# grantjr1842/index-tts

Measured on AMD Instinct MI355X. Metric: synthesised audio seconds per second (IndexTTS-2 infer_v2 hot path), whole job, higher is better.
Workload: dtype f32 (greedy decode + its prefill: exact fp32 MFMA; fp32 accumulate and fp32 activations everywhere) + split-bf16 (fp32 operands as hi+lo bf16, 3 bf16 MFMAs per product) GEMMs, DiT attention and convolutions in s2mel, the latent pass and the vocoder; GPT linear weights STORED as bf16 (rounded once at

## Files before the change

index-tts_amd/csrc/decode.h:

```cpp
#pragma once
#include "common.h"

namespace idxtts {

struct DecodeState {
  int pos;
  int mel_pos;
  int step;
  unsigned arrive;
};

struct SlotState {
  int pos;
  int mel_pos;
  int step;
  int max_step;
  int live;
};

struct DecodeAttnArgs {
  const float* qkv_part = nullptr; int parts = 0; int part_rows = 0;
  const float* qkv_bias = nullptr;
  void* kcache = nullptr; void* vcache = nullptr; int kv16 = 0;
  float* out = nullptr;
  float* out_row = nullptr;
  const int* kstart = nullptr;
  const DecodeState* st = nullptr;
  int B = 0, H = 0, Smax = 0, d = 0;
  float scale = 0.125f;
  int pos_hint = 0;
  int nsplit = 1;
  float* part = nullptr;
  unsigned* cnt = nullptr;
  const SlotState* slot = nullptr;
};
int decode_attn_nsplit(int B, int H);
int decode_attn_forward(const DecodeAttnArgs& a, hipStream_t stream);

struct SampleArgs {
  const float* part = nullptr; int parts = 0; int part_rows = 0;
  const float* bias = nullptr;
  float* logits_out = nullptr;
  unsigned char* seen = nullptr;
  int* finished = nullptr;
  long long* codes = nullptr; int codes_ld = 0;
  int* cur_tok = nullptr;
  const DecodeState* st = nullptr;
  int B = 0, V = 0, stop_token = 0;
  float penalty = 1.0f;
  const long long* forced = nullptr; int forced_ld = 0;
  struct Embed {
    float* x_row = nullptr; float* x_stats = nullptr;
    float* x_frag = nullptr;
    const float* mel_emb = nullptr; const float* mel_pos = nullptr; int d = 0;
    DecodeState* st_rw = nullptr;
  } embed;
};
int sample_greedy_forward(const SampleArgs& a, hipStream_t stream);
int sample_slots_forward(const SampleArgs& a, SlotState* slots, const int* slot_ids, int n, hipStream_t stream);

enum SampleMode { SAMPLE_HF = 1, SAMPLE_ACCEL = 2 };
__host__ __device__ static inline float exp1_draw(const float* noise, unsigned long long seed, size_t idx) {
  if (noise) return noise[idx];
  unsigned long long z = seed + 0x9E3779B97F4A7C15ull * (unsigned long long)(idx + 1);
  z = (z ^ (z >> 30)) * 0xBF58476D1CE4E5B9ull;
  z = (z ^ (z >> 27)) * 0x94D049BB133111EBull;
  z = z ^ (z >> 31);
  const float u = ((float)(z >> 40) + 0.5f) * (1.0f / 16777216.0f);
  return -logf(u);
}
struct SampleWarpArgs {
  SampleArgs base;
  int mode = SAMPLE_HF;
  float temperature = 1.0f;
  int top_k = 0;
  float top_p = 1.0f;
  const float* exp_noise = nullptr;
  unsigned long long seed = 0;
};
int sample_warp_forward(const SampleWarpArgs& a, hipStream_t stream);
struct SlotSampling {
  int mode;
  float temperature;
  int top_k;
  float top_p;
  unsigned long long seed;
  const float* exp_noise;
};
int sample_slots_warp_forward(const SampleArgs& a, SlotState* slots, const SlotSampling* samp, const int* slot_ids, int n,
// ... 48 lines not shown
```

index-tts_amd/csrc/decode.hip:

```cpp
#include <algorithm>
#include <cstdlib>

#include "decode.h"
#include "device_util.h"
#include "prof.h"

namespace idxtts {

__device__ __forceinline__ void decode_attn_finish(const DecodeAttnArgs& p, const int b, const int h, const int z, const int NS, const int tid,
                                                   const float o, const float mx, const float l) {
  const int d = p.d;
  auto put = [&](float val) {
    if (p.out_row) p.out_row[(size_t)b * d + h * 64 + tid] = val;
    else p.out[frag_index(b, h * 64 + tid, d >> 4)] = val;
  };
  if (NS == 1) {
    if (tid < 64) put(l > 0.f ? o / l : 0.f);
    return;
  }
  float* mine = p.part + ((size_t)(b * p.H + h) * NS + z) * 66;
  if (tid < 64) __hip_atomic_store(&mine[tid], o, __ATOMIC_RELAXED, __HIP_MEMORY_SCOPE_AGENT);
  if (tid == 64) __hip_atomic_store(&mine[64], mx, __ATOMIC_RELAXED, __HIP_MEMORY_SCOPE_AGENT);
  if (tid == 65) __hip_atomic_store(&mine[65], l, __ATOMIC_RELAXED, __HIP_MEMORY_SCOPE_AGENT);
  if (!wg_arrive_last(&p.cnt[b * p.H + h], (unsigned)NS) || tid >= 64) return;
  const float* all = p.part + (size_t)(b * p.H + h) * NS * 66;
  float mi[16], li[16], oi[16];
#pragma unroll
  for (int i = 0; i < 16; ++i) {
    const bool on = i < NS;
    mi[i] = on ? __hip_atomic_load(&all[i * 66 + 64], __ATOMIC_RELAXED, __HIP_MEMORY_SCOPE_AGENT) : -1e30f;
    li[i] = on ? __hip_atomic_load(&all[i * 66 + 65], __ATOMIC_RELAXED, __HIP_MEMORY_SCOPE_AGENT) : 0.f;
    oi[i] = on ? __hip_atomic_load(&all[i * 66 + tid], __ATOMIC_RELAXED, __HIP_MEMORY_SCOPE_AGENT) : 0.f;
  }
  float M = -1e30f;
#pragma unroll
  for (int i = 0; i < 16; ++i) M = fmaxf(M, mi[i]);
  float O = 0.f, L = 0.f;
#pragma unroll
  for (int i = 0; i < 16; ++i) {
    const float wgt = li[i] > 0.f ? expf(mi[i] - M) : 0.f;
    O += wgt * oi[i];
    L += wgt * li[i];
  }
  put(L > 0.f ? O / L : 0.f);
}

__device__ __forceinline__ void decode_attn_dead(const DecodeAttnArgs& p, const int b, const int h, const int z, const int tid) {
  if (z != 0 || tid >= 64) return;
  if (p.out_row) p.out_row[(size_t)b * p.d + h * 64 + tid] = 0.f;
  else p.out[frag_index(b, h * 64 + tid, p.d >> 4)] = 0.f;
}

struct KvF32 {
  typedef float E;
  typedef f32x4 G;
  typedef f32x4 Acc;
  typedef f32x4 VNew;
  static constexpr int EPG = 4;
  static constexpr int NACC = 4;
  static constexpr int OUT_UNROLL = 32;
  __device__ static __forceinline__ G zero() { return G{0.f, 0.f, 0.f, 0.f}; }
  __device__ static __forceinline__ float put(E* dst, const bool write, const float x) {
    if (write) *dst = x;
    return x;
  }
  __device__ static __forceinline__ float dot_new(const float (&qv)[64], const float* knew) {
    float dot = 0.f;
#pragma unroll
    for (int i = 0; i < 16; ++i) dot += qv[4 * i] * knew[4 * i] + qv[4 * i + 1] * knew[4 * i + 1] + qv[4 * i + 2] * knew[4 * i + 2] + qv[4 * i + 3] * knew[4 * i + 3];
    return dot;
  }
  __device__ static __forceinline__ float dot_key(const float (&qv)[64], const G (&kk)[16]) {
    float dot = 0.f;
#pragma unroll
    for (int i = 0; i < 16; ++i) dot += qv[4 * i] * kk[i][0] + qv[4 * i + 1] * kk[i][1] + qv[4 * i + 2] * kk[i][2] + qv[4 * i + 3] * kk[i][3];
    return dot;
  }
  __device__ static __forceinline__ VNew vnew_of(const float* vnew, const int l) { return *reinterpret_cast<const f32x4*>(&vnew[4 * l]); }
  __device__ static __forceinline__ void fma(Acc& acc, const float pw, const G v) { acc += pw * v; }
  __device__ static __forceinline__ void fma_new(Acc& acc, const float pw, const VNew vn) { acc += pw * vn; }
  __device__ static __forceinline__ void store(float* dst, const Acc (&a)[4]) { *reinterpret_cast<f32x4*>(dst) = (a[0] + a[1]) + (a[2] + a[3]); }
};
struct KvBf16 {
  typedef unsigned short E;
  typedef u32x4 G;
  struct Acc { float e[8]; };
  typedef const float* VNew;
  static constexpr int EPG = 8;
  static constexpr int NACC = 2;
  static constexpr int OUT_UNROLL = 16;
  __device__ static __forceinline__ G zero() { return G{0u, 0u, 0u, 0u}; }
  __device__ static __forceinline__ float put(E* dst, const bool write, const float x) {
    const unsigned bits = bf16_rne_bits(x);
    if (write) *dst = (unsigned short)bits;
    return __uint_as_float(bits << 16);
  }
  __device__ static __forceinline__ float dot_new(const float (&qv)[64], const float* knew) {
    float dot = 0.f;
#pragma unroll
    for (int i = 0; i < 64; ++i) dot += qv[i] * knew[i];
    return dot;
  }
  __device__ static __forceinline__ float dot_key(const float (&qv)[64], const G (&kk)[8]) {
    float dot = 0.f;
#pragma unroll
    for (int i = 0; i < 8; ++i)
#pragma unroll
      for (int j = 0; j < 4; ++j)
        dot += qv[8 * i + 2 * j] * __uint_as_float(kk[i][j] << 16) + qv[8 * i + 2 * j + 1] * __uint_as_float(kk[i][j] & 0xffff0000u);
    return dot;
  }
  __device__ static __forceinline__ VNew vnew_of(const float* vnew, const int l) { return vnew + 8 * l; }
  __device__ static __forceinline__ void fma(Acc& acc, const float pw, const G v) {
#pragma unroll
    for (int j = 0; j < 4; ++j) {
      acc.e[2 * j] += pw * __uint_as_float(v[j] << 16);
      acc.e[2 * j + 1] += pw * __uint_as_float(v[j] & 0xffff0000u);
    }
  }
  __device__ static __forceinline__ void fma_new(Acc& acc, const float pw, const VNew vn) {
#pragma unroll
    for (int e = 0; e < 8; ++e) acc.e[e] += pw * vn[e];
  }
  __device__ static __forceinline__ void store(float* dst, const Acc (&a)[2]) {
#pragma unroll
    for (int e = 0; e < 8; ++e) dst[e] = a[0].e[e] + a[1].e[e];
  }
};

template <int NT, bool SLOTS, class KV>
__device__ __forceinline__ void decode_attn_body(const DecodeAttnArgs& p) {
  typedef typename KV::G G;
  typedef typename KV::E E;
  constexpr int NW = NT / 64, EPG = KV::EPG, KG = 64 / EPG, LPR = 64 / EPG, NG = NT / LPR, NACC = KV::NACC;
  extern __shared__ __attribute__((aligned(16))) float sm[];
  float* qs = sm;
  float* knew = sm + 64;
  float* vnew = sm + 128;
  float* red = sm + 192;
  float* outp = sm + 256;
  float* pr = sm + 256 + NG * 64;

  const int h = blockIdx.x, b = blockIdx.y, tid = threadIdx.x, wave = tid >> 6, lane = tid & 63;
  int pos;
  if constexpr (SLOTS) {
    if (!p.slot[b].live) { decode_attn_dead(p, b, h, blockIdx.z, tid); return; }
    pos = p.slot[b].pos;
  } else {
    pos = p.st->pos;
  }
  const int d = p.d, Smax = p.Smax;
  G* const kc = static_cast<G*>(p.kcache) + (size_t)(b * p.H + h) * KG * Smax;
  G* const vc = static_cast<G*>(p.vcache) + (size_t)(b * p.H + h) * Smax * LPR;

  const int ks0 = p.kstart ? p.kstart[b] : 0;
  const int NS = gridDim.z, z = blockIdx.z;
  const int chunk = NS > 1 ? (((pos - ks0 + NS) / NS + 15) & ~15) : pos - ks0 + 1;
  const int ks = ks0 + z * chunk;
  const int ke = min(pos, ks + chunk - 1);
  const int grp = tid / LPR, lpr = tid % LPR;
  const int s_first = ks + tid;
  G kk0[KG];
#pragma unroll
  for (int i = 0; i < KG; ++i) kk0[i] = (s_first < pos && s_first <= ke) ? kc[(size_t)i * Smax + s_first] : KV::zero();
  constexpr int VP = 128 / NG;
  G vpre[VP];
#pragma unroll
  for (int j = 0; j < VP; ++j) {
    const int sj = ks + grp + NG * j;
    vpre[j] = (sj < pos && sj <= ke) ? vc[(size_t)sj * LPR + lpr] : KV::zero();
  }

  if (tid < 192) {
    const int which = tid >> 6, dd = tid & 63;
    const int col = which * d + h * 64 + dd;
    const float* row = p.qkv_part + (size_t)b * 3 * d + col;
    const size_t sst = (size_t)p.part_rows * 3 * d;
    float acc = p.qkv_bias ? p.qkv_bias[col] : 0.0f;
    for (int s = 0; s < p.parts; ++s) acc += row[(size_t)s * sst];
    if (which == 0) qs[dd] = acc * p.scale;
    else if (which == 1) knew[dd] = KV::put(reinterpret_cast<E*>(kc + (size_t)(dd / EPG) * Smax + pos) + dd % EPG, z == 0, acc);
    else vnew[dd] = KV::put(reinterpret_cast<E*>(vc + (size_t)pos * LPR) + dd, z == 0, acc);
  }
  __syncthreads();

  const float qlane = qs[lane];
  float qv[64];
#pragma unroll
  for (int i = 0; i < 64; ++i) qv[i] = __int_as_float(__builtin_amdgcn_readlane(__float_as_int(qlane), i));

  float mx = -1e30f;
  if (s_first <= ke) {
    const float dot = s_first == pos ? KV::dot_new(qv, knew) : KV::dot_key(qv, kk0);
    pr[s_first] = dot;
    mx = dot;
  }
  for (int s = s_first + NT; s <= ke; s += NT) {
    float dot;
    if (s == pos) dot = KV::dot_new(qv, knew);
    else {
      G kk[KG];
#pragma unroll
      for (int i = 0; i < KG; ++i) kk[i] = kc[(size_t)i * Smax + s];
      dot = KV::dot_key(qv, kk);
    }
    pr[s] = dot;
    mx = fmaxf(mx, dot);
  }
  mx = wave_max(mx);
  if (lane == 0) red[wave] = mx;
  __syncthreads();
  mx = red[0];
#pragma unroll
  for (int w = 1; w < NW; ++w) mx = fmaxf(mx, red[w]);
  float sum = 0.f;
  for (int s = s_first; s <= ke; s += NT) {
    const float e = expf(pr[s] - mx);
    pr[s] = e;
    sum += e;
  }
  sum = wave_sum(sum);
  if (lane == 0) red[NW + wave] = sum;
  __syncthreads();
  float l = 0.f;
#pragma unroll
  for (int w = 0; w < NW; ++w) l += red[NW + w];

  const typename KV::VNew vn = KV::vnew_of(vnew, lpr);
  typename KV::Acc acc[NACC] = {};
#pragma unroll
  for (int j = 0; j < VP; ++j) {
    const int sj = ks + grp + NG * j;
    if (sj <= ke) {
      if (sj == pos) KV::fma_new(acc[j % NACC], pr[sj], vn);
      else KV::fma(acc[j % NACC], pr[sj], vpre[j]);
    }
  }
  for (int sb = ks + grp + VP * NG; sb <= ke; sb += 8 * NG) {
    G v[8];
#pragma unroll
    for (int j = 0; j < 8; ++j) {
      const int sj = sb + NG * j;
      v[j] = (sj < pos && sj <= ke) ? vc[(size_t)sj * LPR + lpr] : KV::zero();
    }
#pragma unroll
    for (int j = 0; j < 8; ++j) {
      const int sj = sb + NG * j;
      if (sj <= ke) {
        if (sj == pos) KV::fma_new(acc[j % NACC], pr[sj], vn);
        else KV::fma(acc[j % NACC], pr[sj], v[j]);
      }
    }
  }
  KV::store(&outp[grp * 64 + EPG * lpr], acc);
  __syncthreads();
  float o = 0.f;
  if (tid < 64) {
#pragma unroll KV::OUT_UNROLL
    for (int g = 0; g < NG; ++g) o += outp[g * 64 + tid];
  }
  decode_attn_finish(p, b, h, z, NS, tid, o, mx, l);
}

template <int NT, bool SLOTS>
__global__ __launch_bounds__(NT, (NT == 512 ? 4 : 1)) void decode_attn_kernel(const DecodeAttnArgs p) {
  decode_attn_body<NT, SLOTS, KvF32>(p);
}
template <int NT, bool SLOTS>
__global__ __launch_bounds__(NT, (NT == 512 ? 4 : 1)) void decode_attn16_kernel(const DecodeAttnArgs p) {
  decode_attn_body<NT, SLOTS, KvBf16>(p);
}

int decode_attn_nsplit(int B, int H) {
  const int wgs = B * H;
  return wgs <= 128 ? std::max(1, std::min(16, 256 / wgs)) : 1;
}

int decode_attn_forward(const DecodeAttnArgs& a, hipStream_t stream) {
  IDX_CHECK(a.qkv_part && a.kcache && a.vcache && (a.out || a.out_row) && (a.st || a.slot), "null pointer");
  IDX_CHECK(a.d == a.H * 64, "head_dim must be 64");
  constexpr int nt = 512;
  const size_t lds = (size_t)(256 + (nt / (a.kv16 ? 8 : 16)) * 64 + a.Smax) * sizeof(float);
  IDX_CHECK(lds <= 128 * 1024, "Smax too large for the LDS score buffer");
  static DynLdsLimit lds_limit;
  IDX_HIP(lds_limit.set(128 * 1024, decode_attn_kernel<512, false>, decode_attn16_kernel<512, false>, decode_attn_kernel<512, true>, decode_attn16_kernel<512, true>));
  IDX_CHECK(a.nsplit >= 1 && a.nsplit <= 16 && (a.nsplit == 1 || (a.part && a.cnt)), "key split: 1..16 pieces, partial buffer and counters");
  static const int cat = prof_register("decode_attn_kernel"), cat16 = prof_register("decode_attn16_kernel");
  ProfScope prof(a.kv16 ? cat16 : cat, stream, 0.0, (a.kv16 ? 4.0 : 8.0) * a.B * (double)a.pos_hint * a.d);
  const dim3 grid(a.H, a.B, a.nsplit);
  if (a.slot) {
    if (a.kv16) hipLaunchKernelGGL((decode_attn16_kernel<512, true>), grid, dim3(512), lds, stream, a);
    else hipLaunchKernelGGL((decode_attn_kernel<512, true>), grid, dim3(512), lds, stream, a);
  } else {
    if (a.kv16) hipLaunchKernelGGL((decode_attn16_kernel<512, false>), grid, dim3(512), lds, stream, a);
    else hipLaunchKernelGGL((decode_attn_kernel<512, false>), grid, dim3(512), lds, stream, a);
  }
  IDX_LAUNCH_CHECK();
  return 0;
}

__device__ __forceinline__ void greedy_row_argmax(const SampleArgs& p, const int b, const int tid, float* rv, int* ri, float& best_out,
                                                  int& bidx_out) {
  const int wave = tid >> 6, lane = tid & 63;
  const int V = p.V;
  float best = -INFINITY;
  int bidx = 0x7fffffff;
  const unsigned char* seen = p.seen + (size_t)b * V;
  const size_t sst = (size_t)p.part_rows * V;
  const float* prow = p.part + (size_t)b * V;
  for (int v0 = tid; v0 < V; v0 += 4096) {
    float l4[4];
#pragma unroll
    for (int u = 0; u < 4; ++u) {
      const int v = v0 + 1024 * u;
      l4[u] = (v < V && p.bias) ? p.bias[v] : 0.0f;
    }
    for (int s = 0; s < p.parts; ++s) {
#pragma unroll
      for (int u = 0; u < 4; ++u) {
        const int v = v0 + 1024 * u;
        if (v < V) l4[u] += prow[(size_t)s * sst + v];
      }
    }
#pragma unroll
    for (int u = 0; u < 4; ++u) {
      const int v = v0 + 1024 * u;
      if (v >= V) continue;
      float l = l4[u];
      if (p.logits_out) p.logits_out[(size_t)b * V + v] = l;
      if (seen[v]) l = l < 0.f ? l * p.penalty : l / p.penalty;
      if (l > best) { best = l; bidx = v; }
    }
  }
  wave_argmax(best, bidx);
  if (lane == 0) { rv[wave] = best; ri[wave] = bidx; }
  __syncthreads();
  if (tid == 0) argmax_take_waves<16>(best, bidx, rv, ri);
  best_out = best;
  bidx_out = bidx;
}

__device__ __forceinline__ void write_next_input(const SampleArgs& p, const int b, const int tok, const int mel_pos, const int tid) {
  if (p.embed.x_frag) {
    const int d = p.embed.d;
    for (int e = tid; e < d; e += 1024) p.embed.x_frag[frag_index(b, e, d >> 4)] = p.embed.mel_emb[(size_t)tok * d + e] + p.embed.mel_pos[(size_t)mel_pos * d + e];
  } else {
    embed_row_pl<1024>(p.embed.x_row, p.embed.x_stats, b, p.B, p.embed.d, p.embed.mel_emb, p.embed.mel_pos, tok, mel_pos, tid);
  }
// ... 482 lines not shown
```

index-tts_amd/csrc/gpt.hip:

```cpp
#include <algorithm>
#include <cstdlib>
#include <cstring>

#include "gpt.h"
#include "model_util.h"

namespace idxtts {

GPTModel::GPTModel(const idxtts_gpt_config& c) : cfg(c) {}

bool GPTModel::accepts(const std::string& name) const {
  static const char* prefixes[] = {"gpt.h.", "gpt.ln_f.", "final_norm.", "mel_head.", "mel_embedding.", "text_embedding.",
                                   "mel_pos_embedding.", "text_pos_embedding.", "speed_emb."};
  for (const char* p : prefixes)
    if (name.rfind(p, 0) == 0) return true;
  return false;
}

static int upload_stream(DeviceArena& arena, const std::vector<float>& buf, int N, int K, int fmt, Gemv16Weights* gw) {
  gw->N = N; gw->K = K; gw->fmt = fmt;
  if (fmt == WFMT_F32) {
    float* d = nullptr;
    if (arena.upload(buf.data(), buf.size(), &d)) return 1;
    gw->wp = d;
// ... 135 lines not shown
  if (tensor_from(t, arena, "final_norm.weight", {d}, &fn_g) || tensor_from(t, arena, "final_norm.bias", {d}, &fn_b)) return 1;
  const int V = cfg.number_mel_codes;
  HostTensor* hw = nullptr;
  if (need(t, "mel_head.weight", {V, d}, &hw)) return 1;
  std::vector<float> buf(gemv16_packed_floats(V, d));
  pack_gemv16_nk(buf.data(), hw->data.data(), V, d);
  if (upload_stream(arena, buf, V, d, weight_fmt, &head_g)) return 1;
  if (weight_fmt != WFMT_F32 && d % 32 == 0 && upload_stream32(arena, hw->data.data(), V, d, false, weight_fmt, &head_p)) return 1;
  if (tensor_from(t, arena, "mel_head.bias", {V}, &head_b)) return 1;
  if (tensor_from(t, arena, "mel_embedding.weight", {V, d}, &mel_emb)) return 1;
  if (tensor_from(t, arena, "text_embedding.weight", {cfg.number_text_tokens + 1, d}, &text_emb)) return 1;
  if (tensor_from(t, arena, "mel_pos_embedding.emb.weight", {cfg.mel_pos_len, d}, &mel_pos)) return 1;
  if (tensor_from(t, arena, "text_pos_embedding.emb.weight", {cfg.text_pos_len, d}, &text_pos)) return 1;
  return 0;
}

GPTModel::Buffers GPTModel::carve(void* ws, int B, int S, int max_new, size_t prefill_rows) const {
  const int d = cfg.model_dim, V = cfg.number_mel_codes, L = cfg.layers;
  Buffers b;
  Carver c(ws);
  const size_t rows = prefill_rows ? prefill_rows : (size_t)B * S;
  b.x = c.take<float>(rows * d);
  b.h = c.take<float>(rows * d);
  b.qkv = c.take<float>(rows * 3 * d);
  b.att = c.take<float>(rows * d);
  b.ff = c.take<float>(rows * 4 * d);
  b.Smax = max_new > 0 ? ((S + max_new + 3) & ~3) : 0;
  const size_t cache = (size_t)L * kv_layer_bytes(B, b.Smax);
  b.kcache = c.take<char>(cache);
  b.vcache = c.take<char>(cache);
  b.xd = c.take<float>(frag_image_floats(B, d));
  b.frag_off = c.off - frag_image_floats(B, d) * sizeof(float);
  b.hd = c.take<float>(frag_image_floats(B, d));
  b.attd = c.take<float>(frag_image_floats(B, d));
  b.ffd = c.take<float>(frag_image_floats(B, 4 * d));
  b.pl_cnt = c.take<unsigned>((size_t)cdiv(std::max(V, 4 * d), 16));
  b.frag_bytes = c.off - b.frag_off;
  b.xrow = c.take<float>((size_t)B * d);
  b.hrow = c.take<float>((size_t)B * d);
  b.attrow = c.take<float>((size_t)B * d);
  b.ffrow = c.take<float>((size_t)B * 4 * d);
  b.stats = c.take<float>((size_t)cdiv(d, 16) * cdiv(B, 16) * 16 * 2);
  b.pl_slab = c.take<float>(std::max({gemv_pl_slab_floats(3 * d, d, B), gemv_pl_slab_floats(d, d, B), gemv_pl_slab_floats(4 * d, d, B),
                                      gemv_pl_slab_floats(d, 4 * d, B), gemv_pl_slab_floats(V, d, B), (size_t)64}));
  b.qkvd = c.take<float>((size_t)B * 3 * d);
  b.slab = c.take<float>((size_t)8 * B * d);
  b.logits = c.take<float>((size_t)B * V);
  b.seen = c.take<unsigned char>((size_t)B * V);
  b.finished = c.take<int>(B);
  b.cur_tok = c.take<int>(B);
  b.kstart = c.take<int>(B);
  b.ksb_cnt = c.take<unsigned>((size_t)cdiv(d, 16));
  b.attn_cnt = c.take<unsigned>((size_t)B * cfg.heads);
  b.attn_part = c.take<float>((size_t)B * cfg.heads * 16 * 66);
  b.state = c.take<DecodeState>(1);
  b.codes = c.take<long long>((size_t)B * (max_new > 0 ? max_new : 0));
  b.bytes = (c.off + 255) & ~(size_t)255;
  return b;
}

size_t GPTModel::workspace_bytes(int B, int S, int max_new) const { return carve(nullptr, B, S, max_new).bytes; }

int GPTModel::layer_full(int li, const Buffers& w, int B, int S, const int* kstart, bool store_kv, hipStream_t st, const KvScatter* scatter) {
  const bool exact = store_kv && kv_fmt == 0;
  auto mm = [&](const LinearWeights& lw, const GemmArgs& ga) { return exact ? gemm_tn_forward(lw, ga, st) : gemm_forward(lw, ga, st); };
  const GPTLayer& L = layers[li];
  const int d = cfg.model_dim, M = B * S;
  RowsNormArgs n1;
  n1.x_in = w.x; n1.ld_in = d; n1.y = w.h; n1.ld_y = d; n1.M = M; n1.d = d; n1.mode = NORM_LN; n1.g1 = L.ln1_g; n1.b1 = L.ln1_b;
  if (rows_norm_forward(n1, st)) return 1;
  GemmArgs g;
  g.x = w.h; g.ldx = d; g.y = w.qkv; g.ldy = 3 * d; g.M = M;
  if (mm(L.attn_l, g)) return 1;
  if (store_kv && scatter) {
    const size_t per_layer = kv_layer_bytes(scatter->slots, w.Smax);
    if (kv_store_slots(w.qkv, w.kcache + li * per_layer, w.vcache + li * per_layer, kv_fmt, scatter->n, cfg.heads, S, w.Smax, d,
                       scatter->slot_ids, scatter->len, st, scatter->fan)) return 1;
  } else if (store_kv) {
    const size_t per_layer = kv_layer_bytes(B, w.Smax);
    if (kv_store_prefill(w.qkv, w.kcache + li * per_layer, w.vcache + li * per_layer, kv_fmt, B, cfg.heads, S, w.Smax, d, st)) return 1;
  }
  AttnArgs a;
  a.q = w.qkv; a.k = w.qkv + d; a.v = w.qkv + 2 * d; a.o = w.att;
  a.q_bs = a.k_bs = a.v_bs = (long)S * 3 * d; a.o_bs = (long)S * d;
  a.q_ts = a.k_ts = a.v_ts = 3 * d; a.o_ts = d;
  a.B = B; a.H = cfg.heads; a.Sq = S; a.Sk = S; a.causal = 1; a.kstart = kstart; a.scale = 0.125f;
  a.split_bf16 = !exact && get_gemm_mode() == GEMM_BF16X3;
  if (flash_attn_forward(a, st)) return 1;
  GemmArgs p;
  p.x = w.att; p.ldx = d; p.y = w.x; p.ldy = d; p.res = w.x; p.ldr = d; p.M = M;
  if (mm(L.proj_l, p)) return 1;
  RowsNormArgs n2 = n1;
  n2.g1 = L.ln2_g; n2.b1 = L.ln2_b;
  if (rows_norm_forward(n2, st)) return 1;
  GemmArgs f1;
  f1.x = w.h; f1.ldx = d; f1.y = w.ff; f1.ldy = 4 * d; f1.M = M; f1.act = ACT_GELU_NEW;
  if (mm(L.fc_l, f1)) return 1;
  GemmArgs f2;
  f2.x = w.ff; f2.ldx = 4 * d; f2.y = w.x; f2.ldy = d; f2.res = w.x; f2.ldr = d; f2.M = M;
  if (mm(L.fc2_l, f2)) return 1;
  return 0;
}

int GPTModel::head_logits(const Buffers& w, int B, const float* x, int ldx, bool x_frag, hipStream_t st) {
  const int V = cfg.number_mel_codes, d = cfg.model_dim;
  const bool pl = use_pl(B);
  RowsNormArgs n;
// ... 16 lines not shown
int GPTModel::head_and_sample(const Buffers& w, int B, const float* x, int ldx, bool x_frag, float penalty, int codes_ld,
                              float* logits_out, hipStream_t st) {
  const int V = cfg.number_mel_codes, d = cfg.model_dim;
  const bool pl = use_pl(B);
  if (head_logits(w, B, x, ldx, x_frag, st)) return 1;
  if (w.beam_tail) {
    BeamState bs = w.beam;
    bs.penalty = penalty;
    return beam_scores_forward(bs, st) || beam_select_forward(bs, st) || beam_reorder_forward(bs, st);
  }
  SampleArgs s;
  s.part = w.logits; s.parts = 1; s.part_rows = B; s.bias = nullptr; s.logits_out = logits_out;
  s.seen = w.seen; s.finished = w.finished; s.codes = w.codes; s.codes_ld = codes_ld; s.cur_tok = w.cur_tok;
  s.st = w.state; s.B = B; s.V = V; s.stop_token = cfg.stop_mel_token; s.penalty = penalty;
  s.forced = w.forced; s.forced_ld = w.forced_ld;
  if (w.slots) {
    if (pl) { s.embed.x_row = w.xrow; s.embed.x_stats = w.stats; } else s.embed.x_frag = w.xd;
    s.embed.mel_emb = mel_emb; s.embed.mel_pos = mel_pos; s.embed.d = d;
    if (w.slot_samp) return sample_slots_warp_forward(s, w.slots, w.slot_samp, nullptr, B, st);
    return sample_slots_forward(s, w.slots, nullptr, B, st);
  }
  if (fused_tail(w)) {
    if (pl) { s.embed.x_row = w.xrow; s.embed.x_stats = w.stats; } else s.embed.x_frag = w.xd;
    s.embed.mel_emb = mel_emb; s.embed.mel_pos = mel_pos; s.embed.d = d; s.embed.st_rw = w.state;
  }
  if (w.samp.mode != 0) {
    const idxtts_sampling& r = w.samp;
    SampleWarpArgs sw;
    sw.base = s; sw.mode = r.mode; sw.temperature = r.temperature; sw.top_k = r.top_k; sw.top_p = r.top_p;
    sw.exp_noise = r.exp_noise; sw.seed = r.seed;
    return sample_warp_forward(sw, st);
  }
  return sample_greedy_forward(s, st);
}

bool GPTModel::use_pl(int B) const { return weight_fmt != WFMT_F32 && B >= get_decode_plane_rows() && cfg.model_dim % 32 == 0 && head_p.wp; }
bool GPTModel::fused_tail(const Buffers& w) const { return w.slots || (w.samp.mode == 0 && !w.beam_tail); }

int GPTModel::decode_step_pl(const Buffers& w, int B, float penalty, int codes_ld, float* logits_base, int pos_hint, hipStream_t st) {
  const int d = cfg.model_dim, T = d / 16;
  const size_t per_layer = kv_layer_bytes(B, w.Smax);
  const bool fused = fused_tail(w);
  if (!fused && embed_step_pl(w.xrow, w.stats, B, d, mel_emb, mel_pos, w.cur_tok, w.state, st)) return 1;
  for (int li = 0; li < cfg.layers; ++li) {
    const GPTLayer& L = layers[li];
    GemvPLArgs qa;
    qa.x = w.xrow; qa.ldx = d; qa.rows = B; qa.colsum = L.attn_u; qa.bias = L.attn_c; qa.stats_in = w.stats; qa.stats_tiles = T;
    qa.y = w.qkvd; qa.ldy = 3 * d; qa.slab = w.pl_slab; qa.counters = w.pl_cnt;
    if (gemv_pl_forward(L.attn_p, qa, st)) return 1;
    DecodeAttnArgs da;
    da.qkv_part = w.qkvd; da.parts = 1; da.part_rows = B; da.qkv_bias = nullptr;
    da.kcache = w.kcache + li * per_layer; da.vcache = w.vcache + li * per_layer; da.kv16 = kv_fmt; da.out_row = w.attrow; da.kstart = w.kstart;
    da.st = w.state; da.B = B; da.H = cfg.heads; da.Smax = w.Smax; da.d = d; da.scale = 0.125f;
    da.nsplit = decode_attn_nsplit(B, cfg.heads); da.part = w.attn_part; da.cnt = w.attn_cnt; da.slot = w.slots;
    da.pos_hint = pos_hint;
    if (decode_attn_forward(da, st)) return 1;
    GemvPLArgs pa;
    pa.x = w.attrow; pa.ldx = d; pa.rows = B; pa.bias = L.proj_l.bias; pa.res = w.xrow; pa.y = w.xrow; pa.ldy = d; pa.stats_out = w.stats;
    pa.slab = w.pl_slab; pa.counters = w.pl_cnt;
    if (gemv_pl_forward(L.proj_p, pa, st)) return 1;
    GemvPLArgs fa;
    fa.x = w.xrow; fa.ldx = d; fa.rows = B; fa.colsum = L.fc_u; fa.bias = L.fc_c; fa.stats_in = w.stats; fa.stats_tiles = T; fa.act = 1; fa.y = w.ffrow; fa.ldy = 4 * d;
    fa.slab = w.pl_slab; fa.counters = w.pl_cnt;
    if (gemv_pl_forward(L.fc_p, fa, st)) return 1;
    GemvPLArgs fb;
    fb.x = w.ffrow; fb.ldx = 4 * d; fb.rows = B; fb.bias = L.fc2_l.bias; fb.res = w.xrow; fb.y = w.xrow; fb.ldy = d; fb.stats_out = w.stats;
    fb.slab = w.pl_slab; fb.counters = w.pl_cnt;
    if (gemv_pl_forward(L.fc2_p, fb, st)) return 1;
  }
  if (head_and_sample(w, B, w.xrow, d, false, penalty, codes_ld, logits_base, st)) return 1;
  return fused ? 0 : advance_state(w.state, st);
}

int GPTModel::decode_step(const Buffers& w, int B, float penalty, int codes_ld, float* logits_base, int pos_hint, hipStream_t st) {
  if (use_pl(B)) return decode_step_pl(w, B, penalty, codes_ld, logits_base, pos_hint, st);
  const int d = cfg.model_dim;
  const size_t per_layer = kv_layer_bytes(B, w.Smax);
  const bool fused = fused_tail(w);
  if (!fused && embed_step(w.xd, B, d, mel_emb, mel_pos, w.cur_tok, w.state, st)) return 1;
  for (int li = 0; li < cfg.layers; ++li) {
    const GPTLayer& L = layers[li];
    GemvFXArgs qa;
    qa.xf = w.xd; qa.rows = B; qa.colsum = L.attn_u; qa.bias = L.attn_c; qa.y = w.qkvd; qa.ldy = 3 * d;
    if (gemv_fx_forward(L.attn_g, qa, st)) return 1;
    DecodeAttnArgs da;
    da.qkv_part = w.qkvd; da.parts = 1; da.part_rows = B; da.qkv_bias = nullptr;
    da.kcache = w.kcache + li * per_layer; da.vcache = w.vcache + li * per_layer; da.kv16 = kv_fmt; da.out = w.attd; da.kstart = w.kstart;
    da.st = w.state; da.B = B; da.H = cfg.heads; da.Smax = w.Smax; da.d = d; da.scale = 0.125f;
    da.nsplit = decode_attn_nsplit(B, cfg.heads); da.part = w.attn_part; da.cnt = w.attn_cnt; da.slot = w.slots;
    da.pos_hint = pos_hint;
    if (decode_attn_forward(da, st)) return 1;
    GemvFXArgs pa;
    pa.xf = w.attd; pa.rows = B; pa.bias = L.proj_l.bias; pa.res = w.xd; pa.y = w.xd; pa.y_frag = 1;
    if (gemv_fx_forward(L.proj_g, pa, st)) return 1;
    GemvFXArgs fa;
    fa.xf = w.xd; fa.rows = B; fa.colsum = L.fc_u; fa.bias = L.fc_c; fa.act = 1; fa.y = w.ffd; fa.y_frag = 1;
    if (gemv_fx_forward(L.fc_g, fa, st)) return 1;
    GemvFXArgs fb;
    fb.xf = w.ffd; fb.rows = B;
    const int ksb = gemv_fx_ksb(L.fc2_g.N, L.fc2_g.K);
    if (ksb > 1) {
      fb.ksb = ksb; fb.slab = w.slab; fb.ksb_counters = w.ksb_cnt;
      fb.bias = L.fc2_l.bias; fb.res = w.xd; fb.y = w.xd; fb.y_frag = 1;
      if (gemv_fx_forward(L.fc2_g, fb, st)) return 1;
    } else {
      fb.bias = L.fc2_l.bias; fb.res = w.xd; fb.y = w.xd; fb.y_frag = 1;
      if (gemv_fx_forward(L.fc2_g, fb, st)) return 1;
    }
  }
  if (head_and_sample(w, B, w.xd, d, true, penalty, codes_ld, logits_base, st)) return 1;
  return fused ? 0 : advance_state(w.state, st);
}

int GPTModel::capture_step(const Buffers& w, int B, float penalty, int codes_ld, hipStream_t st, StepGraph* g) {
  IDX_HIP(hipStreamBeginCapture(st, hipStreamCaptureModeThreadLocal));
  const int rc = decode_step(w, B, penalty, codes_ld, nullptr, 0, st);
  const hipError_t e = hipStreamEndCapture(st, &g->graph);
  if (rc) return 1;
  IDX_HIP(e);
  IDX_HIP(hipGraphInstantiate(&g->exec, g->graph, nullptr, nullptr, 0));
  return 0;
}

int GPTModel::call_stream(hipStream_t user, hipStream_t* st) {
  *st = user;
  if (user) return 0;
  if (!own_stream) IDX_HIP(hipStreamCreateWithFlags(&own_stream, hipStreamNonBlocking));
  IDX_HIP(hipStreamSynchronize(user));
  *st = own_stream;
  return 0;
}

int GPTModel::run_generation(const Buffers& w, const float* inputs_embeds, const int* pad_left_host, int B, int fan, int P, int max_new,
                             float penalty, float* logits_out, bool graph, hipGraphExec_t exec, StepGraph* captured, const int* poll,
                             int poll_n, int poll_every, int* steps_done, hipStream_t st) {
  const int d = cfg.model_dim, V = cfg.number_mel_codes, S = P + 1, R = B * fan;
  std::vector<int> kstart(R, 0);
  for (int r = 0; r < R; ++r) {
    kstart[r] = pad_left_host ? pad_left_host[r / fan] : 0;
    IDX_CHECK(kstart[r] >= 0 && kstart[r] < P, "pad_left out of range");
  }
  IDX_HIP(hipMemcpyAsync(w.kstart, kstart.data(), R * sizeof(int), hipMemcpyHostToDevice, st));
// ... 433 lines not shown
```

Measured before the change: 188.8.

## Rewrite decode attention as persistent per-wave 64-key chunks with balanced work split

Replaces the per-(head,row,split) workgroup decode attention with a persistent grid sized to the CU count. Each wave handles one 64-key chunk of one (row, head) pair, and the work is balanced across blocks using a prefix sum of live chunk counts per row. Partials are merged by the last-arriving wave through an online softmax. This removes the LDS score buffer and the fixed split heuristic, so the split adapts to each row's actual length and dead slots cost nothing. In exchange it adds per-chunk atomic counters and partial traffic, recomputes q for every chunk, and requires a partial buffer that grows with Smax.

Result: slower. 182.3 (-3.4%).

```diff
diff --git a/index-tts_amd/csrc/decode.h b/index-tts_amd/csrc/decode.h
--- a/index-tts_amd/csrc/decode.h
+++ b/index-tts_amd/csrc/decode.h
@@ -29,12 +29,11 @@
   int B = 0, H = 0, Smax = 0, d = 0;
   float scale = 0.125f;
   int pos_hint = 0;
-  int nsplit = 1;
   float* part = nullptr;
   unsigned* cnt = nullptr;
   const SlotState* slot = nullptr;
 };
-int decode_attn_nsplit(int B, int H);
+size_t decode_attn_part_floats(int B, int H, int Smax);
 int decode_attn_forward(const DecodeAttnArgs& a, hipStream_t stream);
 
 struct SampleArgs {
diff --git a/index-tts_amd/csrc/decode.hip b/index-tts_amd/csrc/decode.hip
--- a/index-tts_amd/csrc/decode.hip
+++ b/index-tts_amd/csrc/decode.hip
@@ -7,99 +7,57 @@
 
 namespace idxtts {
 
-__device__ __forceinline__ void decode_attn_finish(const DecodeAttnArgs& p, const int b, const int h, const int z, const int NS, const int tid,
-                                                   const float o, const float mx, const float l) {
-  const int d = p.d;
-  auto put = [&](float val) {
-    if (p.out_row) p.out_row[(size_t)b * d + h * 64 + tid] = val;
-    else p.out[frag_index(b, h * 64 + tid, d >> 4)] = val;
-  };
-  if (NS == 1) {
-    if (tid < 64) put(l > 0.f ? o / l : 0.f);
-    return;
-  }
-  float* mine = p.part + ((size_t)(b * p.H + h) * NS + z) * 66;
-  if (tid < 64) __hip_atomic_store(&mine[tid], o, __ATOMIC_RELAXED, __HIP_MEMORY_SCOPE_AGENT);
-  if (tid == 64) __hip_atomic_store(&mine[64], mx, __ATOMIC_RELAXED, __HIP_MEMORY_SCOPE_AGENT);
-  if (tid == 65) __hip_atomic_store(&mine[65], l, __ATOMIC_RELAXED, __HIP_MEMORY_SCOPE_AGENT);
-  if (!wg_arrive_last(&p.cnt[b * p.H + h], (unsigned)NS) || tid >= 64) return;
-  const float* all = p.part + (size_t)(b * p.H + h) * NS * 66;
-  float mi[16], li[16], oi[16];
-#pragma unroll
-  for (int i = 0; i < 16; ++i) {
-    const bool on = i < NS;
-    mi[i] = on ? __hip_atomic_load(&all[i * 66 + 64], __ATOMIC_RELAXED, __HIP_MEMORY_SCOPE_AGENT) : -1e30f;
-    li[i] = on ? __hip_atomic_load(&all[i * 66 + 65], __ATOMIC_RELAXED, __HIP_MEMORY_SCOPE_AGENT) : 0.f;
-    oi[i] = on ? __hip_atomic_load(&all[i * 66 + tid], __ATOMIC_RELAXED, __HIP_MEMORY_SCOPE_AGENT) : 0.f;
-  }
-  float M = -1e30f;
-#pragma unroll
-  for (int i = 0; i < 16; ++i) M = fmaxf(M, mi[i]);
-  float O = 0.f, L = 0.f;
-#pragma unroll
-  for (int i = 0; i < 16; ++i) {
-    const float wgt = li[i] > 0.f ? expf(mi[i] - M) : 0.f;
-    O += wgt * oi[i];
-    L += wgt * li[i];
-  }
-  put(L > 0.f ? O / L : 0.f);
-}
-
-__device__ __forceinline__ void decode_attn_dead(const DecodeAttnArgs& p, const int b, const int h, const int z, const int tid) {
-  if (z != 0 || tid >= 64) return;
-  if (p.out_row) p.out_row[(size_t)b * p.d + h * 64 + tid] = 0.f;
-  else p.out[frag_index(b, h * 64 + tid, p.d >> 4)] = 0.f;
-}
+constexpr int DA_NT = 512, DA_NW = DA_NT / 64;
+constexpr int DA_GRAN = 64;
+constexpr int DA_PF = 66;
+constexpr int DA_MAX_ROWS = 512;
+
+size_t decode_attn_part_floats(int B, int H, int Smax) { return (size_t)B * H * cdiv(Smax, DA_GRAN) * DA_PF; }
 
 struct KvF32 {
   typedef float E;
   typedef f32x4 G;
   typedef f32x4 Acc;
-  typedef f32x4 VNew;
   static constexpr int EPG = 4;
-  static constexpr int NACC = 4;
-  static constexpr int OUT_UNROLL = 32;
+  static constexpr int NACC = 2;
+  static constexpr int VPRE = 4;
   __device__ static __forceinline__ G zero() { return G{0.f, 0.f, 0.f, 0.f}; }
-  __device__ static __forceinline__ float put(E* dst, const bool write, const float x) {
-    if (write) *dst = x;
+  __device__ static __forceinline__ float put(E* dst, const float x) {
+    *dst = x;
     return x;
   }
-  __device__ static __forceinline__ float dot_new(const float (&qv)[64], const float* knew) {
-    float dot = 0.f;
-#pragma unroll
-    for (int i = 0; i < 16; ++i) dot += qv[4 * i] * knew[4 * i] + qv[4 * i + 1] * knew[4 * i + 1] + qv[4 * i + 2] * knew[4 * i + 2] + qv[4 * i + 3] * knew[4 * i + 3];
-    return dot;
-  }
+  __device__ static __forceinline__ G pack(const float (&x)[4]) { return G{x[0], x[1], x[2], x[3]}; }
   __device__ static __forceinline__ float dot_key(const float (&qv)[64], const G (&kk)[16]) {
     float dot = 0.f;
 #pragma unroll
     for (int i = 0; i < 16; ++i) dot += qv[4 * i] * kk[i][0] + qv[4 * i + 1] * kk[i][1] + qv[4 * i + 2] * kk[i][2] + qv[4 * i + 3] * kk[i][3];
     return dot;
   }
-  __device__ static __forceinline__ VNew vnew_of(const float* vnew, const int l) { return *reinterpret_cast<const f32x4*>(&vnew[4 * l]); }
   __device__ static __forceinline__ void fma(Acc& acc, const float pw, const G v) { acc += pw * v; }
-  __device__ static __forceinline__ void fma_new(Acc& acc, const float pw, const VNew vn) { acc += pw * vn; }
-  __device__ static __forceinline__ void store(float* dst, const Acc (&a)[4]) { *reinterpret_cast<f32x4*>(dst) = (a[0] + a[1]) + (a[2] + a[3]); }
+  __device__ static __forceinline__ void sum(float (&o)[4], const Acc (&a)[2]) {
+    const f32x4 t = a[0] + a[1];
+#pragma unroll
+    for (int e = 0; e < 4; ++e) o[e] = t[e];
+  }
 };
 struct KvBf16 {
   typedef unsigned short E;
   typedef u32x4 G;
   struct Acc { float e[8]; };
-  typedef const float* VNew;
   static constexpr int EPG = 8;
   static constexpr int NACC = 2;
-  static constexpr int OUT_UNROLL = 16;
+  static constexpr int VPRE = 4;
   __device__ static __forceinline__ G zero() { return G{0u, 0u, 0u, 0u}; }
-  __device__ static __forceinline__ float put(E* dst, const bool write, const float x) {
+  __device__ static __forceinline__ float put(E* dst, const float x) {
     const unsigned bits = bf16_rne_bits(x);
-    if (write) *dst = (unsigned short)bits;
+    *dst = (unsigned short)bits;
     return __uint_as_float(bits << 16);
   }
-  __device__ static __forceinline__ float dot_new(const float (&qv)[64], const float* knew) {
-    float dot = 0.f;
-#pragma unroll
-    for (int i = 0; i < 64; ++i) dot += qv[i] * knew[i];
-    return dot;
+  __device__ static __forceinline__ G pack(const float (&x)[8]) {
+    G g;
+#pragma unroll
+    for (int j = 0; j < 4; ++j) g[j] = (__float_as_uint(x[2 * j]) >> 16) | (__float_as_uint(x[2 * j + 1]) & 0xffff0000u);
+    return g;
   }
   __device__ static __forceinline__ float dot_key(const float (&qv)[64], const G (&kk)[8]) {
     float dot = 0.f;
@@ -110,7 +68,6 @@
         dot += qv[8 * i + 2 * j] * __uint_as_float(kk[i][j] << 16) + qv[8 * i + 2 * j + 1] * __uint_as_float(kk[i][j] & 0xffff0000u);
     return dot;
   }
-  __device__ static __forceinline__ VNew vnew_of(const float* vnew, const int l) { return vnew + 8 * l; }
   __device__ static __forceinline__ void fma(Acc& acc, const float pw, const G v) {
 #pragma unroll
     for (int j = 0; j < 4; ++j) {
@@ -118,182 +75,229 @@
       acc.e[2 * j + 1] += pw * __uint_as_float(v[j] & 0xffff0000u);
     }
   }
-  __device__ static __forceinline__ void fma_new(Acc& acc, const float pw, const VNew vn) {
-#pragma unroll
-    for (int e = 0; e < 8; ++e) acc.e[e] += pw * vn[e];
-  }
-  __device__ static __forceinline__ void store(float* dst, const Acc (&a)[2]) {
-#pragma unroll
-    for (int e = 0; e < 8; ++e) dst[e] = a[0].e[e] + a[1].e[e];
+  __device__ static __forceinline__ void sum(float (&o)[8], const Acc (&a)[2]) {
+#pragma unroll
+    for (int e = 0; e < 8; ++e) o[e] = a[0].e[e] + a[1].e[e];
   }
 };
 
-template <int NT, bool SLOTS, class KV>
+__device__ __forceinline__ void decode_attn_put(const DecodeAttnArgs& p, const int b, const int col, const float val) {
+  if (p.out_row) p.out_row[(size_t)b * p.d + col] = val;
+  else p.out[frag_index(b, col, p.d >> 4)] = val;
+}
+
+template <bool SLOTS, class KV>
 __device__ __forceinline__ void decode_attn_body(const DecodeAttnArgs& p) {
   typedef typename KV::G G;
   typedef typename KV::E E;
-  constexpr int NW = NT / 64, EPG = KV::EPG, KG = 64 / EPG, LPR = 64 / EPG, NG = NT / LPR, NACC = KV::NACC;
-  extern __shared__ __attribute__((aligned(16))) float sm[];
-  float* qs = sm;
-  float* knew = sm + 64;
-  float* vnew = sm + 128;
-  float* red = sm + 192;
-  float* outp = sm + 256;
-  float* pr = sm + 256 + NG * 64;
-
-  const int h = blockIdx.x, b = blockIdx.y, tid = threadIdx.x, wave = tid >> 6, lane = tid & 63;
-  int pos;
-  if constexpr (SLOTS) {
-    if (!p.slot[b].live) { decode_attn_dead(p, b, h, blockIdx.z, tid); return; }
-    pos = p.slot[b].pos;
-  } else {
-    pos = p.st->pos;
-  }
-  const int d = p.d, Smax = p.Smax;
-  G* const kc = static_cast<G*>(p.kcache) + (size_t)(b * p.H + h) * KG * Smax;
-  G* const vc = static_cast<G*>(p.vcache) + (size_t)(b * p.H + h) * Smax * LPR;
-
-  const int ks0 = p.kstart ? p.kstart[b] : 0;
-  const int NS = gridDim.z, z = blockIdx.z;
-  const int chunk = NS > 1 ? (((pos - ks0 + NS) / NS + 15) & ~15) : pos - ks0 + 1;
-  const int ks = ks0 + z * chunk;
-  const int ke = min(pos, ks + chunk - 1);
-  const int grp = tid / LPR, lpr = tid % LPR;
-  const int s_first = ks + tid;
-  G kk0[KG];
-#pragma unroll
-  for (int i = 0; i < KG; ++i) kk0[i] = (s_first < pos && s_first <= ke) ? kc[(size_t)i * Smax + s_first] : KV::zero();
-  constexpr int VP = 128 / NG;
-  G vpre[VP];
-#pragma unroll
-  for (int j = 0; j < VP; ++j) {
-    const int sj = ks + grp + NG * j;
-    vpre[j] = (sj < pos && sj <= ke) ? vc[(size_t)sj * LPR + lpr] : KV::zero();
-  }
-
-  if (tid < 192) {
-    const int which = tid >> 6, dd = tid & 63;
-    const int col = which * d + h * 64 + dd;
-    const float* row = p.qkv_part + (size_t)b * 3 * d + col;
+  constexpr int EPG = KV::EPG, KG = 64 / EPG, LPR = 64 / EPG, NGW = 64 / LPR, NV = DA_GRAN / NGW, NACC = KV::NACC, VPRE = KV::VPRE;
+  static_assert(NGW == EPG, "a lane group's index selects the head dim a lane hands on");
+  __shared__ int s_incl[DA_MAX_ROWS];
+  __shared__ int s_pos[DA_MAX_ROWS];
+  __shared__ int s_ks[DA_MAX_ROWS];
+  const int tid = threadIdx.x, wave = tid >> 6, lane = tid & 63;
+  const int B = p.B, H = p.H, d = p.d, Smax = p.Smax;
+  const int Gmax = (Smax + DA_GRAN - 1) / DA_GRAN;
+
+  if (wave == 0) {
+    int carry = 0;
+    for (int r0 = 0; r0 < B; r0 += 64) {
+      const int r = r0 + lane;
+      int pos = 0, ks0 = 0, g = 0;
+      if (r < B) {
+        bool live = true;
+        ks0 = p.kstart ? p.kstart[r] : 0;
+        if constexpr (SLOTS) { live = p.slot[r].live != 0; pos = p.slot[r].pos; }
+        else pos = p.st->pos;
+        if (live && ks0 >= 0 && pos >= ks0 && pos < Smax) g = (pos - ks0) / DA_GRAN + 1;
+      }
+      int inc = g;
+#pragma unroll
+      for (int off = 1; off < 64; off <<= 1) {
+        const int t = __shfl_up(inc, off);
+        if (lane >= off) inc += t;
+      }
+      inc += carry;
+      if (r < B) { s_incl[r] = inc; s_pos[r] = pos; s_ks[r] = ks0; }
+      carry = __shfl(inc, 63);
+    }
+  }
+  __syncthreads();
+
+  const int T = H * s_incl[B - 1];
+  const int W = min(T, (int)gridDim.x);
+  int run0 = 0, run1 = 0;
+  if ((int)blockIdx.x < W) {
+    run0 = (int)((long long)blockIdx.x * T / W);
+    run1 = (int)((long long)(blockIdx.x + 1) * T / W);
+  }
+
+  for (int f = run0 + wave; f < run1; f += DA_NW) {
+    int b = 0;
+    for (int r0 = 0; r0 < B; r0 += 64) {
+      const int r = r0 + lane;
+      b += __popcll(__ballot(r < B && s_incl[r] * H <= f));
+    }
+    b = __builtin_amdgcn_readfirstlane(b);
+    if (b >= B) break;
+    const int gbase = b ? __builtin_amdgcn_readfirstlane(s_incl[b - 1]) : 0, gb = __builtin_amdgcn_readfirstlane(s_incl[b]) - gbase;
+    if (gb <= 0) break;
+    const int rem = f - gbase * H, h = rem / gb, j = rem - h * gb;
+    const int pos = __builtin_amdgcn_readfirstlane(s_pos[b]);
+    const int gs = __builtin_amdgcn_readfirstlane(s_ks[b]) + DA_GRAN * j;
+    const bool last = j == gb - 1;
+    const int pair = b * H + h;
+    G* const kc = static_cast<G*>(p.kcache) + (size_t)pair * KG * Smax;
+    G* const vc = static_cast<G*>(p.vcache) + (size_t)pair * Smax * LPR;
+    const G* const kg = kc + gs;
+    const G* const vg0 = vc + (size_t)gs * LPR;
+    const int grp = lane / LPR, lpr = lane % LPR;
+    const int s = gs + lane;
+
+    G kk[KG];
+#pragma unroll
+    for (int i = 0; i < KG; ++i) kk[i] = s < pos ? (kg + (size_t)i * Smax)[(unsigned)lane] : KV::zero();
+    G v[NV];
+#pragma unroll
+    for (int jj = 0; jj < VPRE; ++jj) {
+      const int sj = gs + grp + NGW * jj;
+      v[jj] = sj < pos ? (vg0 + NGW * LPR * jj)[(unsigned)lane] : KV::zero();
+    }
+
     const size_t sst = (size_t)p.part_rows * 3 * d;
-    float acc = p.qkv_bias ? p.qkv_bias[col] : 0.0f;
-    for (int s = 0; s < p.parts; ++s) acc += row[(size_t)s * sst];
-    if (which == 0) qs[dd] = acc * p.scale;
-    else if (which == 1) knew[dd] = KV::put(reinterpret_cast<E*>(kc + (size_t)(dd / EPG) * Smax + pos) + dd % EPG, z == 0, acc);
-    else vnew[dd] = KV::put(reinterpret_cast<E*>(vc + (size_t)pos * LPR) + dd, z == 0, acc);
-  }
-  __syncthreads();
-
-  const float qlane = qs[lane];
-  float qv[64];
-#pragma unroll
-  for (int i = 0; i < 64; ++i) qv[i] = __int_as_float(__builtin_amdgcn_readlane(__float_as_int(qlane), i));
-
-  float mx = -1e30f;
-  if (s_first <= ke) {
-    const float dot = s_first == pos ? KV::dot_new(qv, knew) : KV::dot_key(qv, kk0);
-    pr[s_first] = dot;
-    mx = dot;
-  }
-  for (int s = s_first + NT; s <= ke; s += NT) {
-    float dot;
-    if (s == pos) dot = KV::dot_new(qv, knew);
-    else {
-      G kk[KG];
-#pragma unroll
-      for (int i = 0; i < KG; ++i) kk[i] = kc[(size_t)i * Smax + s];
-      dot = KV::dot_key(qv, kk);
-    }
-    pr[s] = dot;
-    mx = fmaxf(mx, dot);
-  }
-  mx = wave_max(mx);
-  if (lane == 0) red[wave] = mx;
-  __syncthreads();
-  mx = red[0];
-#pragma unroll
-  for (int w = 1; w < NW; ++w) mx = fmaxf(mx, red[w]);
-  float sum = 0.f;
-  for (int s = s_first; s <= ke; s += NT) {
-    const float e = expf(pr[s] - mx);
-    pr[s] = e;
-    sum += e;
-  }
-  sum = wave_sum(sum);
-  if (lane == 0) red[NW + wave] = sum;
-  __syncthreads();
-  float l = 0.f;
-#pragma unroll
-  for (int w = 0; w < NW; ++w) l += red[NW + w];
-
-  const typename KV::VNew vn = KV::vnew_of(vnew, lpr);
-  typename KV::Acc acc[NACC] = {};
-#pragma unroll
-  for (int j = 0; j < VP; ++j) {
-    const int sj = ks + grp + NG * j;
-    if (sj <= ke) {
-      if (sj == pos) KV::fma_new(acc[j % NACC], pr[sj], vn);
-      else KV::fma(acc[j % NACC], pr[sj], vpre[j]);
-    }
-  }
-  for (int sb = ks + grp + VP * NG; sb <= ke; sb += 8 * NG) {
-    G v[8];
-#pragma unroll
-    for (int j = 0; j < 8; ++j) {
-      const int sj = sb + NG * j;
-      v[j] = (sj < pos && sj <= ke) ? vc[(size_t)sj * LPR + lpr] : KV::zero();
-    }
-#pragma unroll
-    for (int j = 0; j < 8; ++j) {
-      const int sj = sb + NG * j;
-      if (sj <= ke) {
-        if (sj == pos) KV::fma_new(acc[j % NACC], pr[sj], vn);
-        else KV::fma(acc[j % NACC], pr[sj], v[j]);
-      }
-    }
-  }
-  KV::store(&outp[grp * 64 + EPG * lpr], acc);
-  __syncthreads();
-  float o = 0.f;
-  if (tid < 64) {
-#pragma unroll KV::OUT_UNROLL
-    for (int g = 0; g < NG; ++g) o += outp[g * 64 + tid];
-  }
-  decode_attn_finish(p, b, h, z, NS, tid, o, mx, l);
-}
-
-template <int NT, bool SLOTS>
-__global__ __launch_bounds__(NT, (NT == 512 ? 4 : 1)) void decode_attn_kernel(const DecodeAttnArgs p) {
-  decode_attn_body<NT, SLOTS, KvF32>(p);
-}
-template <int NT, bool SLOTS>
-__global__ __launch_bounds__(NT, (NT == 512 ? 4 : 1)) void decode_attn16_kernel(const DecodeAttnArgs p) {
-  decode_attn_body<NT, SLOTS, KvBf16>(p);
-}
-
-int decode_attn_nsplit(int B, int H) {
-  const int wgs = B * H;
-  return wgs <= 128 ? std::max(1, std::min(16, 256 / wgs)) : 1;
+    const float* row = p.qkv_part + (size_t)b * 3 * d + h * 64 + lane;
+    float qa = p.qkv_bias ? p.qkv_bias[h * 64 + lane] : 0.0f;
+    for (int t = 0; t < p.parts; ++t) qa += row[(size_t)t * sst];
+    const float qlane = qa * p.scale;
+    float klane = 0.f, vlane = 0.f;
+    if (last) {
+      float ka = p.qkv_bias ? p.qkv_bias[d + h * 64 + lane] : 0.0f, va = p.qkv_bias ? p.qkv_bias[2 * d + h * 64 + lane] : 0.0f;
+      for (int t = 0; t < p.parts; ++t) { ka += row[(size_t)t * sst + d]; va += row[(size_t)t * sst + 2 * d]; }
+      klane = KV::put(reinterpret_cast<E*>(kc + (size_t)(lane / EPG) * Smax + pos) + lane % EPG, ka);
+      vlane = KV::put(reinterpret_cast<E*>(vc + (size_t)pos * LPR) + lane, va);
+    }
+    float qv[64];
+#pragma unroll
+    for (int i = 0; i < 64; ++i) qv[i] = __int_as_float(__builtin_amdgcn_readlane(__float_as_int(qlane), i));
+
+    float dot = KV::dot_key(qv, kk);
+    if (last) {
+      const float dn = wave_sum(qlane * klane);
+      if (s == pos) dot = dn;
+    }
+    __builtin_amdgcn_sched_barrier(0);
+#pragma unroll
+    for (int jj = VPRE; jj < NV; ++jj) {
+      const int sj = gs + grp + NGW * jj;
+      v[jj] = sj < pos ? (vg0 + NGW * LPR * jj)[(unsigned)lane] : KV::zero();
+    }
+    const bool on = s <= pos;
+    const float m = wave_max(on ? dot : -1e30f);
+    const float e = on ? expf(dot - m) : 0.f;
+    const float l = wave_sum(e);
+
+    if (last) {
+      float vn[EPG];
+#pragma unroll
+      for (int i = 0; i < EPG; ++i) vn[i] = __shfl(vlane, EPG * lpr + i);
+      const G vg = KV::pack(vn);
+#pragma unroll
+      for (int jj = 0; jj < NV; ++jj)
+        if (gs + grp + NGW * jj == pos) v[jj] = vg;
+    }
+    typename KV::Acc acc[NACC] = {};
+#pragma unroll
+    for (int jj = 0; jj < NV; ++jj) KV::fma(acc[jj % NACC], __shfl(e, grp + NGW * jj), v[jj]);
+    float o[EPG];
+    KV::sum(o, acc);
+#pragma unroll
+    for (int off = LPR; off < 64; off <<= 1)
+#pragma unroll
+      for (int i = 0; i < EPG; ++i) o[i] += __shfl_xor(o[i], off);
+    float mine = o[0];
+#pragma unroll
+    for (int i = 1; i < EPG; ++i) mine = grp == i ? o[i] : mine;
+    const int dd = EPG * lpr + grp;
+
+    if (gb == 1) {
+      decode_attn_put(p, b, h * 64 + dd, l > 0.f ? mine / l : 0.f);
+      continue;
+    }
+    float* const all = p.part + (size_t)pair * Gmax * DA_PF;
+    float* const part = all + (size_t)j * DA_PF;
+    __hip_atomic_store(&part[dd], mine, __ATOMIC_RELAXED, __HIP_MEMORY_SCOPE_AGENT);
+    if (lane == 0) {
+      __hip_atomic_store(&part[64], m, __ATOMIC_RELAXED, __HIP_MEMORY_SCOPE_AGENT);
+      __hip_atomic_store(&part[65], l, __ATOMIC_RELAXED, __HIP_MEMORY_SCOPE_AGENT);
+    }
+    asm volatile("s_waitcnt vmcnt(0)" ::: "memory");
+    int is_last = 0;
+    if (lane == 0) {
+      const unsigned old = __hip_atomic_fetch_add(&p.cnt[pair], 1u, __ATOMIC_RELAXED, __HIP_MEMORY_SCOPE_AGENT);
+      is_last = old == (unsigned)gb - 1u;
+      if (is_last) __hip_atomic_store(&p.cnt[pair], 0u, __ATOMIC_RELAXED, __HIP_MEMORY_SCOPE_AGENT);
+    }
+    is_last = __builtin_amdgcn_readfirstlane(is_last);
+    asm volatile("" ::: "memory");
+    if (!is_last) continue;
+    float M = -1e30f, L = 0.f, O = 0.f;
+    for (int i0 = 0; i0 < gb; i0 += 8) {
+      float mi[8], li[8], oi[8];
+#pragma unroll
+      for (int i = 0; i < 8; ++i) {
+        const bool in = i0 + i < gb;
+        const float* pi = all + (size_t)(i0 + i) * DA_PF;
+        mi[i] = in ? __hip_atomic_load(&pi[64], __ATOMIC_RELAXED, __HIP_MEMORY_SCOPE_AGENT) : -1e30f;
+        li[i] = in ? __hip_atomic_load(&pi[65], __ATOMIC_RELAXED, __HIP_MEMORY_SCOPE_AGENT) : 0.f;
+        oi[i] = in ? __hip_atomic_load(&pi[lane], __ATOMIC_RELAXED, __HIP_MEMORY_SCOPE_AGENT) : 0.f;
+      }
+#pragma unroll
+      for (int i = 0; i < 8; ++i) {
+        if (i0 + i < gb) {
+          const float mn = fmaxf(M, mi[i]);
+          const float wa = expf(M - mn), wb = expf(mi[i] - mn);
+          O = O * wa + oi[i] * wb;
+          L = L * wa + li[i] * wb;
+          M = mn;
+        }
+      }
+    }
+    decode_attn_put(p, b, h * 64 + lane, L > 0.f ? O / L : 0.f);
+  }
+
+  for (int i = blockIdx.x * DA_NT + tid; i < B * d; i += gridDim.x * DA_NT) {
+    const int r = i / d;
+    if (s_incl[r] == (r ? s_incl[r - 1] : 0)) decode_attn_put(p, r, i - r * d, 0.f);
+  }
+}
+
+template <bool SLOTS>
+__global__ __launch_bounds__(DA_NT, 4) void decode_attn_kernel(const DecodeAttnArgs p) {
+  decode_attn_body<SLOTS, KvF32>(p);
+}
+template <bool SLOTS>
+__global__ __launch_bounds__(DA_NT, 4) void decode_attn16_kernel(const DecodeAttnArgs p) {
+  decode_attn_body<SLOTS, KvBf16>(p);
 }
 
 int decode_attn_forward(const DecodeAttnArgs& a, hipStream_t stream) {
-  IDX_CHECK(a.qkv_part && a.kcache && a.vcache && (a.out || a.out_row) && (a.st || a.slot), "null pointer");
+  IDX_CHECK(a.qkv_part && a.kcache && a.vcache && (a.out || a.out_row) && (a.st || a.slot) && a.part && a.cnt, "null pointer");
   IDX_CHECK(a.d == a.H * 64, "head_dim must be 64");
-  constexpr int nt = 512;
-  const size_t lds = (size_t)(256 + (nt / (a.kv16 ? 8 : 16)) * 64 + a.Smax) * sizeof(float);
-  IDX_CHECK(lds <= 128 * 1024, "Smax too large for the LDS score buffer");
-  static DynLdsLimit lds_limit;
-  IDX_HIP(lds_limit.set(128 * 1024, decode_attn_kernel<512, false>, decode_attn16_kernel<512, false>, decode_attn_kernel<512, true>, decode_attn16_kernel<512, true>));
-  IDX_CHECK(a.nsplit >= 1 && a.nsplit <= 16 && (a.nsplit == 1 || (a.part && a.cnt)), "key split: 1..16 pieces, partial buffer and counters");
+  IDX_CHECK(a.B >= 1 && a.B <= DA_MAX_ROWS && a.Smax >= 1, "1 <= rows <= 512");
+  static const int cus = [] {
+    int dev = 0, n = 0;
+    if (hipGetDevice(&dev) != hipSuccess || hipDeviceGetAttribute(&n, hipDeviceAttributeMultiprocessorCount, dev) != hipSuccess || n <= 0) n = 256;
+    return n;
+  }();
   static const int cat = prof_register("decode_attn_kernel"), cat16 = prof_register("decode_attn16_kernel");
   ProfScope prof(a.kv16 ? cat16 : cat, stream, 0.0, (a.kv16 ? 4.0 : 8.0) * a.B * (double)a.pos_hint * a.d);
-  const dim3 grid(a.H, a.B, a.nsplit);
+  const dim3 grid((unsigned)std::min<long long>(cus, (long long)a.B * a.H * cdiv(a.Smax, DA_GRAN)));
   if (a.slot) {
-    if (a.kv16) hipLaunchKernelGGL((decode_attn16_kernel<512, true>), grid, dim3(512), lds, stream, a);
-    else hipLaunchKernelGGL((decode_attn_kernel<512, true>), grid, dim3(512), lds, stream, a);
+    if (a.kv16) hipLaunchKernelGGL((decode_attn16_kernel<true>), grid, dim3(DA_NT), 0, stream, a);
+    else hipLaunchKernelGGL((decode_attn_kernel<true>), grid, dim3(DA_NT), 0, stream, a);
   } else {
-    if (a.kv16) hipLaunchKernelGGL((decode_attn16_kernel<512, false>), grid, dim3(512), lds, stream, a);
-    else hipLaunchKernelGGL((decode_attn_kernel<512, false>), grid, dim3(512), lds, stream, a);
+    if (a.kv16) hipLaunchKernelGGL((decode_attn16_kernel<false>), grid, dim3(DA_NT), 0, stream, a);
+    else hipLaunchKernelGGL((decode_attn_kernel<false>), grid, dim3(DA_NT), 0, stream, a);
   }
   IDX_LAUNCH_CHECK();
   return 0;
diff --git a/index-tts_amd/csrc/gpt.hip b/index-tts_amd/csrc/gpt.hip
--- a/index-tts_amd/csrc/gpt.hip
+++ b/index-tts_amd/csrc/gpt.hip
@@ -211,7 +211,7 @@
   b.kstart = c.take<int>(B);
   b.ksb_cnt = c.take<unsigned>((size_t)cdiv(d, 16));
   b.attn_cnt = c.take<unsigned>((size_t)B * cfg.heads);
-  b.attn_part = c.take<float>((size_t)B * cfg.heads * 16 * 66);
+  b.attn_part = c.take<float>(decode_attn_part_floats(B, cfg.heads, b.Smax));
   b.state = c.take<DecodeState>(1);
   b.codes = c.take<long long>((size_t)B * (max_new > 0 ? max_new : 0));
   b.bytes = (c.off + 255) & ~(size_t)255;
@@ -334,7 +334,7 @@
     da.qkv_part = w.qkvd; da.parts = 1; da.part_rows = B; da.qkv_bias = nullptr;
     da.kcache = w.kcache + li * per_layer; da.vcache = w.vcache + li * per_layer; da.kv16 = kv_fmt; da.out_row = w.attrow; da.kstart = w.kstart;
     da.st = w.state; da.B = B; da.H = cfg.heads; da.Smax = w.Smax; da.d = d; da.scale = 0.125f;
-    da.nsplit = decode_attn_nsplit(B, cfg.heads); da.part = w.attn_part; da.cnt = w.attn_cnt; da.slot = w.slots;
+    da.part = w.attn_part; da.cnt = w.attn_cnt; da.slot = w.slots;
     da.pos_hint = pos_hint;
     if (decode_attn_forward(da, st)) return 1;
     GemvPLArgs pa;
@@ -369,7 +369,7 @@
     da.qkv_part = w.qkvd; da.parts = 1; da.part_rows = B; da.qkv_bias = nullptr;
     da.kcache = w.kcache + li * per_layer; da.vcache = w.vcache + li * per_layer; da.kv16 = kv_fmt; da.out = w.attd; da.kstart = w.kstart;
     da.st = w.state; da.B = B; da.H = cfg.heads; da.Smax = w.Smax; da.d = d; da.scale = 0.125f;
-    da.nsplit = decode_attn_nsplit(B, cfg.heads); da.part = w.attn_part; da.cnt = w.attn_cnt; da.slot = w.slots;
+    da.part = w.attn_part; da.cnt = w.attn_cnt; da.slot = w.slots;
     da.pos_hint = pos_hint;
     if (decode_attn_forward(da, st)) return 1;
     GemvFXArgs pa;
```
